# Niccolo-Ajroldi/plainLM

Hardware: AMD Instinct MI355X
Metric: tokens/sec fwd+bwd (160M, seq=1024, bf16) (higher is better)
Workload: dtype bf16

## Files before the change

### plainlm_amd/csrc/attn_causal.hip

```cpp
#include "plm_device.h"

#include <type_traits>

#include "attn_common.h"

template <int RB>
__device__ __forceinline__ void attn_block2(int T, int nh, int& tile, int& h, int& b) {
  const int ntile = (T + RB - 1) / RB;
  const int nbh = gridDim.x / ntile;
  const int bh = blockIdx.x % nbh;
  tile = blockIdx.x / nbh;
  h = bh % nh;
  b = bh / nh;
}

constexpr int ATTN_DMA_PER_STAGE = 4;
constexpr int ATTN_DMA_STATS = 2;
static_assert(ATTN_DMA_PER_STAGE == 2 * 2, "stage() = two TileDma::issue calls of two instructions each");

#define ATTN_DEFER_LOG2 8.0f
#define PLM_ATTN_TRACE_SETTER plm_dbg_attn_trace_causal
ATTN_TRACE_DECL()
#ifdef PLM_ATTN_ONEPASS_ABLATION
static __device__ float* g_onepass_buf = nullptr;
static __device__ int g_onepass_mode = 0;
extern "C" int plm_dbg_attn_onepass(float* buf, int mode) {
  if (hipMemcpyToSymbol(HIP_SYMBOL(g_onepass_buf), &buf, sizeof(buf)) != hipSuccess) return -1;
  return (int)hipMemcpyToSymbol(HIP_SYMBOL(g_onepass_mode), &mode, sizeof(mode));
}
#define ONEPASS_LDS 8192
#else
#define ONEPASS_LDS 0
#endif

enum { QB_OFF = 0, QB_UM = 1, QB_MASK = 2 };

template <int NST>
__global__ __launch_bounds__(256, 2) void attn_fwd_causal_kernel(const uint16_t* __restrict__ qkv, uint16_t* __restrict__ out,
                                                                 float* __restrict__ lse, int T, int nh) {
  constexpr int KT = 64;
  constexpr int TILE = KT * 128;
  constexpr int QB = 256;
  __shared__ __attribute__((aligned(1024))) char smem[NST * 2 * TILE];

  int tile_, h, b;
  attn_block2<QB>(T, nh, tile_, h, b);
  const int qt = (T + QB - 1) / QB - 1 - tile_;
  const int dm = nh * HD, ld = 3 * dm;
  const int t = threadIdx.x, lane = t & 63;
  const int wave = __builtin_amdgcn_readfirstlane(t >> 6);
  const int l31 = lane & 31, hi = lane >> 5;
  const int q0 = qt * QB;
  const int r0[2] = {q0 + 32 * wave, q0 + 32 * (7 - wave)};
  const uint16_t* base = qkv + (int64_t)b * T * ld + h * HD;
  const float c2 = 0.125f * LOG2E;

  const int kv_hi = min(T, q0 + QB);
  const int jt_hi = (kv_hi + KT - 1) / KT;
  constexpr int jt_lo = 0;
  const int n = jt_hi;

  TileDma dma;
  dma.init(wave, lane, ld);
  auto stage = [&](int slot, int jt) {
    const int kv0 = jt * KT;
    const uint16_t* src = base + (int64_t)kv0 * ld;
    if (kv0 + KT <= T) {
      dma.issue_full(smem + slot * 2 * TILE, src + dm, wave);
      dma.issue_full(smem + slot * 2 * TILE + TILE, src + 2 * dm, wave);
    } else {
      dma.issue(smem + slot * 2 * TILE, src + dm, ld, T - 1 - kv0, wave);
      dma.issue(smem + slot * 2 * TILE + TILE, src + 2 * dm, ld, T - 1 - kv0, wave);
    }
  };

  if (n > 0) stage(0, jt_lo);

  bf16x8_t qf[2][4];
#pragma unroll
  for (int qb = 0; qb < 2; ++qb) {
    const int qrow = r0[qb] + l31;
    const bool qvalid = qrow < T;
#pragma unroll
    for (int ks = 0; ks < 4; ++ks) qf[qb][ks] = qvalid ? ld_bf16x8(base + (int64_t)qrow * ld + ks * 16 + hi * 8) : zero_bf16x8();
  }
#pragma unroll
  for (int qb = 0; qb < 2; ++qb) asm volatile("; q fragments resident" ::"v"(qf[qb][0]), "v"(qf[qb][1]), "v"(qf[qb][2]), "v"(qf[qb][3]));
  asm volatile("s_waitcnt vmcnt(0)" ::: "memory");
#pragma unroll
  for (int i = 1; i < NST - 1; ++i)
    if (i < n) stage(i, jt_lo + i);

  f32x16_t o[2][2];
  float mc[2], lsum[2];
#pragma unroll
  for (int qb = 0; qb < 2; ++qb) {
    zero16(o[qb][0]);
    zero16(o[qb][1]);
    mc[qb] = -INFINITY;
    lsum[qb] = 0.f;
  }

  auto soft_pv = [&](int qb_, f32x16_t (&s)[2], const bf16x8_t (&vfr)[2][4], int kv0, auto mask_tag) {
    constexpr bool MASK = decltype(mask_tag)::value;
    const int qb = qb_;
    const int c_hi = r0[qb] + l31 - kv0 - 4 * hi;
    float tmax = -INFINITY;
#pragma unroll
    for (int kb = 0; kb < 2; ++kb)
#pragma unroll
      for (int r = 0; r < 16; ++r) {
        if (MASK) {
          const int c = kb * 32 + (r & 3) + 8 * (r >> 2);
          if (c > c_hi) s[kb][r] = -INFINITY;
        }
        tmax = fmaxf(tmax, s[kb][r]);
      }
    {
      float t_lo, t_hi;
      half_pair(tmax, t_lo, t_hi);
      tmax = fmaxf(t_lo, t_hi);
    }
    const float tm = tmax * c2;
    const bool need = tm > mc[qb] + ATTN_DEFER_LOG2;
    if (__builtin_amdgcn_ballot_w64(need) != 0ull) {
      const float mn = fmaxf(mc[qb], tm);
      const float alpha = fast_exp2(mc[qb] - ((mn == -INFINITY) ? 0.f : mn));
      mc[qb] = mn;
      lsum[qb] *= alpha;
#pragma unroll
      for (int db = 0; db < 2; ++db)
#pragma unroll
        for (int r = 0; r < 16; ++r) o[qb][db][r] *= alpha;
    }
    const float mref = (MASK && mc[qb] == -INFINITY) ? 0.f : mc[qb];
    float ps[4] = {0.f, 0.f, 0.f, 0.f};
    bf16x8_t pf[4];
#pragma unroll
    for (int kb = 0; kb < 2; ++kb)
#pragma unroll
      for (int r = 0; r < 16; ++r) {
        const float p = fast_exp2(__builtin_fmaf(s[kb][r], c2, -mref));
        ps[r & 3] += p;
        pf[kb * 2 + (r >> 3)][r & 7] = f2bf(p);
      }
    lsum[qb] += (ps[0] + ps[1]) + (ps[2] + ps[3]);
#pragma unroll
    for (int db = 0; db < 2; ++db)
#pragma unroll
      for (int sp = 0; sp < 4; ++sp) o[qb][db] = mfma32(vfr[db][sp], pf[sp], o[qb][db]);
  };

  auto compute = [&](int kv0, const char* sK, const char* sV, auto m0_tag, auto m1_tag) {
    constexpr int M0 = decltype(m0_tag)::value, M1 = decltype(m1_tag)::value;
    bf16x8_t kfr[2][4];
#pragma unroll
    for (int kb = 0; kb < 2; ++kb)
#pragma unroll
      for (int ks = 0; ks < 4; ++ks) kfr[kb][ks] = frag_rows(sK, kb * 32 + l31, ks, hi);
    f32x16_t s[2][2];
#pragma unroll
    for (int qb = 0; qb < 2; ++qb) {
      if ((qb == 0 ? M0 : M1) == QB_OFF) continue;
#pragma unroll
      for (int kb = 0; kb < 2; ++kb) {
        zero16(s[qb][kb]);
#pragma unroll
        for (int ks = 0; ks < 4; ++ks) s[qb][kb] = mfma32(kfr[kb][ks], qf[qb][ks], s[qb][kb]);
      }
    }
    __builtin_amdgcn_sched_barrier(0);
    bf16x8_t vfr[2][4];
#pragma unroll
    for (int db = 0; db < 2; ++db)
#pragma unroll
      for (int sp = 0; sp < 4; ++sp) vfr[db][sp] = frag_cols(sV, db, (sp >> 1) * 32 + (sp & 1) * 16 + 4 * hi, lane);
    if (M0 == QB_UM) soft_pv(0, s[0], vfr, kv0, std::false_type{});
    if (M0 == QB_MASK) soft_pv(0, s[0], vfr, kv0, std::true_type{});
    if (M1 == QB_UM) soft_pv(1, s[1], vfr, kv0, std::false_type{});
    if (M1 == QB_MASK) soft_pv(1, s[1], vfr, kv0, std::true_type{});
  };

  int i = 0, slot = 0;
  auto run = [&](int jt_end, auto m0_tag, auto m1_tag, bool active) {
    for (; jt_lo + i < jt_end; ++i) {
      const int rem = min(NST - 2, n - 1 - i);
      if (NST >= 4 && rem >= 2) attn_wait_vm<2 * ATTN_DMA_PER_STAGE>();
      else if (NST >= 3 && rem == 1) attn_wait_vm<ATTN_DMA_PER_STAGE>();
      else attn_wait_vm<0>();
      attn_barrier();
      if (i + NST - 1 < n) stage(slot == 0 ? NST - 1 : slot - 1, jt_lo + i + NST - 1);
      if (active) compute((jt_lo + i) * KT, smem + slot * 2 * TILE, smem + slot * 2 * TILE + TILE, m0_tag, m1_tag);
      slot = (slot + 1 == NST) ? 0 : slot + 1;
    }
  };
  using OFF_ = std::integral_constant<int, QB_OFF>;
  using UM_ = std::integral_constant<int, QB_UM>;
  using MK_ = std::integral_constant<int, QB_MASK>;
  const int a0 = min(jt_hi, r0[0] / KT), e0 = min(jt_hi, r0[0] / KT + 1);
  const int a1 = min(jt_hi, r0[1] / KT), e1 = min(jt_hi, r0[1] / KT + 1);
  run(a0, UM_{}, UM_{}, true);
  run(e0, MK_{}, UM_{}, true);
  run(a1, OFF_{}, UM_{}, true);
  run(e1, OFF_{}, MK_{}, true);
  run(jt_hi, OFF_{}, OFF_{}, false);

  const RowStage rs{smem + (n % NST) * 2 * TILE + wave * 4096, lane};
#pragma unroll
  for (int qb = 0; qb < 2; ++qb) {
    const int qrow = r0[qb] + l31;
    float l_lo, l_hi;
    half_pair(lsum[qb], l_lo, l_hi);
    const float ltot = l_lo + l_hi;
    const float inv = 1.f / ltot;
#pragma unroll
    for (int db = 0; db < 2; ++db)
#pragma unroll
      for (int g = 0; g < 4; ++g) {
        bf16x4_t v;
#pragma unroll
        for (int e = 0; e < 4; ++e) v[e] = f2bf(o[qb][db][4 * g + e] * inv);
        rs.put(l31, hi, db * 4 + g, v);
      }
    if (qrow < T && hi == 0) lse[((int64_t)b * nh + h) * T + qrow] = mc[qb] + __builtin_amdgcn_logf(ltot);
    rs.flush(out + (int64_t)b * T * dm, dm, r0[qb], T, h * HD);
  }
}

template <int NST>
__global__ __launch_bounds__(256, 2) void attn_bwd_dq_causal_kernel(const uint16_t* __restrict__ qkv, const uint16_t* __restrict__ out,
                                                              const uint16_t* __restrict__ dout, const float* __restrict__ lse,
                                                              float* __restrict__ delta, const float* __restrict__ rcos,
                                                              const float* __restrict__ rsin, uint16_t* __restrict__ dqkv, int T, int nh,
                                                              float dsign) {
  constexpr int KT = 64;
  constexpr int TILE = KT * 128;
  constexpr int QB = 256;
  __shared__ __attribute__((aligned(1024))) char smem[NST * 2 * TILE];

  int tile_, h, b;
  attn_block2<QB>(T, nh, tile_, h, b);
  const int qt = (T + QB - 1) / QB - 1 - tile_;
  const int dm = nh * HD, ld = 3 * dm;
  const int t = threadIdx.x, lane = t & 63;
  const int wave = __builtin_amdgcn_readfirstlane(t >> 6);
  const int l31 = lane & 31, hi = lane >> 5;
  const int q0 = qt * QB;
  const int r0[2] = {q0 + 32 * wave, q0 + 32 * (7 - wave)};
  const uint16_t* base = qkv + (int64_t)b * T * ld + h * HD;
  const float scale = 0.125f, c2 = scale * LOG2E;

  const int kv_hi = min(T, q0 + QB);
  const int jt_hi = (kv_hi + KT - 1) / KT;
  constexpr int jt_lo = 0;
  const int n = jt_hi;

  TileDma dma;
  dma.init(wave, lane, ld);
  auto stage = [&](int slot, int jt) {
    const int kv0 = jt * KT;
    const uint16_t* src = base + (int64_t)kv0 * ld;
    if (kv0 + KT <= T) {
      dma.issue_full(smem + slot * 2 * TILE, src + dm, wave);
      dma.issue_full(smem + slot * 2 * TILE + TILE, src + 2 * dm, wave);
    } else {
      dma.issue(smem + slot * 2 * TILE, src + dm, ld, T - 1 - kv0, wave);
      dma.issue(smem + slot * 2 * TILE + TILE, src + 2 * dm, ld, T - 1 - kv0, wave);
    }
  };

  if (n > 0) stage(0, jt_lo);

  bf16x8_t qf[2][4], dof[2][4];
  float Lq[2], Dq[2];
#pragma unroll
  for (int qb = 0; qb < 2; ++qb) {
    const int qrow = r0[qb] + l31;
    const bool qvalid = qrow < T;
#pragma unroll
    for (int ks = 0; ks < 4; ++ks) {
      const int d0 = ks * 16 + hi * 8;
      qf[qb][ks] = qvalid ? ld_bf16x8(base + (int64_t)qrow * ld + d0) : zero_bf16x8();
      dof[qb][ks] = qvalid ? ld_bf16x8(dout + ((int64_t)b * T + qrow) * dm + h * HD + d0) : zero_bf16x8();
    }
    Lq[qb] = 0.f;
    float part = 0.f;
    if (qvalid) {
      Lq[qb] = lse[((int64_t)b * nh + h) * T + qrow];
#pragma unroll
      for (int ks = 0; ks < 4; ++ks) {
        const bf16x8_t o8 = ld_bf16x8(out + ((int64_t)b * T + qrow) * dm + h * HD + ks * 16 + hi * 8);
#pragma unroll
        for (int e = 0; e < 8; ++e) part += bf2f(o8[e]) * bf2f(dof[qb][ks][e]);
      }
    }
    float d_lo, d_hi;
    half_pair(part, d_lo, d_hi);
    Dq[qb] = d_lo + d_hi;
  }
#pragma unroll
  for (int qb = 0; qb < 2; ++qb)
    asm volatile("; q/dO fragments resident" ::"v"(qf[qb][0]), "v"(qf[qb][1]), "v"(qf[qb][2]), "v"(qf[qb][3]), "v"(dof[qb][0]), "v"(dof[qb][1]),
                 "v"(dof[qb][2]), "v"(dof[qb][3]), "v"(Lq[qb]), "v"(Dq[qb]));
  asm volatile("s_waitcnt vmcnt(0)" ::: "memory");
#pragma unroll
  for (int i = 1; i < NST - 1; ++i)
    if (i < n) stage(i, jt_lo + i);

  f32x16_t dq[2][2];
#pragma unroll
  for (int qb = 0; qb < 2; ++qb) {
    zero16(dq[qb][0]);
    zero16(dq[qb][1]);
  }

  auto block = [&](int qb_, int kb, const bf16x8_t (&kfr)[4], const bf16x8_t (&vfr)[4], const bf16x8_t (&ktr)[2][2], int kv0, auto mask_tag) {
    constexpr bool MASK = decltype(mask_tag)::value;
    const int qb = qb_;
    const int c_hi = r0[qb] + l31 - kv0 - 4 * hi;
    f32x16_t s, dp;
    zero16(s);
    zero16(dp);
#pragma unroll
    for (int ks = 0; ks < 4; ++ks) {
      s = mfma32(kfr[ks], qf[qb][ks], s);
      dp = mfma32(vfr[ks], dof[qb][ks], dp);
    }
    bf16x8_t dsf[2];
#pragma unroll
    for (int r = 0; r < 16; ++r) {
      float p = fast_exp2(__builtin_fmaf(s[r], c2, -Lq[qb]));
      if (MASK) {
        const int c = kb * 32 + (r & 3) + 8 * (r >> 2);
        p = (c <= c_hi) ? p : 0.f;
      }
      dsf[r >> 3][r & 7] = f2bf(p * (dp[r] - Dq[qb]));
    }
#pragma unroll
    for (int s2 = 0; s2 < 2; ++s2)
#pragma unroll
      for (int db = 0; db < 2; ++db) dq[qb][db] = mfma32(ktr[db][s2], dsf[s2], dq[qb][db]);
  };

  auto compute = [&](int kv0, const char* sK, const char* sV, auto m0_tag, auto m1_tag) {
    constexpr int M0 = decltype(m0_tag)::value, M1 = decltype(m1_tag)::value;
#pragma unroll
    for (int kb = 0; kb < 2; ++kb) {
      __builtin_amdgcn_sched_barrier(0);
      bf16x8_t kfr[4], vfr[4], ktr[2][2];
#pragma unroll
      for (int ks = 0; ks < 4; ++ks) {
        kfr[ks] = frag_rows(sK, kb * 32 + l31, ks, hi);
        vfr[ks] = frag_rows(sV, kb * 32 + l31, ks, hi);
      }
#pragma unroll
      for (int s2 = 0; s2 < 2; ++s2)
#pragma unroll
        for (int db = 0; db < 2; ++db) ktr[db][s2] = frag_cols(sK, db, kb * 32 + s2 * 16 + 4 * hi, lane);
      if (M0 == QB_UM) block(0, kb, kfr, vfr, ktr, kv0, std::false_type{});
      if (M0 == QB_MASK) block(0, kb, kfr, vfr, ktr, kv0, std::true_type{});
      if (M1 == QB_UM) block(1, kb, kfr, vfr, ktr, kv0, std::false_type{});
      if (M1 == QB_MASK) block(1, kb, kfr, vfr, ktr, kv0, std::true_type{});
    }
  };

  int i = 0, slot = 0;
  auto run = [&](int jt_end, auto m0_tag, auto m1_tag, bool active) {
    for (; jt_lo + i < jt_end; ++i) {
      const int rem = min(NST - 2, n - 1 - i);
      if (NST >= 4 && rem >= 2) attn_wait_vm<2 * ATTN_DMA_PER_STAGE>();
      else if (NST >= 3 && rem == 1) attn_wait_vm<ATTN_DMA_PER_STAGE>();
      else attn_wait_vm<0>();
      attn_barrier();
      if (i + NST - 1 < n) stage(slot == 0 ? NST - 1 : slot - 1, jt_lo + i + NST - 1);
      if (active) compute((jt_lo + i) * KT, smem + slot * 2 * TILE, smem + slot * 2 * TILE + TILE, m0_tag, m1_tag);
      slot = (slot + 1 == NST) ? 0 : slot + 1;
    }
  };
  using OFF_ = std::integral_constant<int, QB_OFF>;
  using UM_ = std::integral_constant<int, QB_UM>;
  using MK_ = std::integral_constant<int, QB_MASK>;
  const int a0 = min(jt_hi, r0[0] / KT), e0 = min(jt_hi, r0[0] / KT + 1);
  const int a1 = min(jt_hi, r0[1] / KT), e1 = min(jt_hi, r0[1] / KT + 1);
  run(a0, UM_{}, UM_{}, true);
  run(e0, MK_{}, UM_{}, true);
  run(a1, OFF_{}, UM_{}, true);
  run(e1, OFF_{}, MK_{}, true);
  run(jt_hi, OFF_{}, OFF_{}, false);

  const RowStage rs{smem + (n % NST) * 2 * TILE + wave * 4096, lane};
#pragma unroll
  for (int qb = 0; qb < 2; ++qb) {
    if (r0[qb] + l31 < T && hi == 0) delta[((int64_t)b * nh + h) * T + r0[qb] + l31] = Dq[qb] * dsign;
#pragma unroll
    for (int db = 0; db < 2; ++db)
#pragma unroll
      for (int g = 0; g < 4; ++g) {
        bf16x4_t ov;
#pragma unroll
        for (int e = 0; e < 4; ++e) ov[e] = f2bf(dq[qb][db][4 * g + e] * scale);
        rs.put(l31, hi, db * 4 + g, ov);
      }
    rs.flush_rot(dqkv + (int64_t)b * T * ld, ld, r0[qb], T, h * HD, rcos, rsin);
  }
}

template <int NST, bool DOC>
__device__ __forceinline__ void attn_bwd_dkdv_body(char* smem, const uint16_t* __restrict__ qkv, const uint16_t* __restrict__ dout,
                                                   const float* __restrict__ lse, const float* __restrict__ ndelta,
                                                   const float* __restrict__ rcos, const float* __restrict__ rsin,
                                                   const int32_t* __restrict__ doc_end, uint16_t* __restrict__ dqkv, int T, int nh, int b, int h,
                                                   int kv0, int jq_plan, unsigned long long* trace_t = nullptr) {
  constexpr int QT = 64;
  constexpr int TILE = QT * 128;
  constexpr int STAGE = 2 * TILE + 512;
  constexpr int NQB = 2;
  const int dm = nh * HD, ld = 3 * dm;
  const int t = threadIdx.x, lane = t & 63;
  const int wave = __builtin_amdgcn_readfirstlane(t >> 6);
  const int l31 = lane & 31, hi = lane >> 5;
  constexpr int qoff = 0;
  const int kvw0 = kv0 + 32 * wave;
  const int kvrow = kvw0 + l31;
  const bool kvalid = kvrow < T;
  const uint16_t* base = qkv + (int64_t)b * T * ld + h * HD;
  const uint16_t* dobase = dout + (int64_t)b * T * dm + h * HD;
  const float* lrow = lse + ((int64_t)b * nh + h) * T;
  const float* drow = ndelta + ((int64_t)b * nh + h) * T;
  const float scale = 0.125f, c2 = scale * LOG2E;

  const int nqt = (T + QT - 1) / QT;
  const int jq_lo = kv0 / QT;
  const int jq_hi = DOC ? jq_plan : nqt;
  const int n = jq_hi - jq_lo;

  TileDma dma, dmad;
  dma.init(wave, lane, ld);
  dmad.init(wave, lane, dm);
  auto stage = [&](int slot, int jq) {
    const int qt0 = jq * QT;
    char* dst = smem + slot * STAGE;
    if (qt0 + QT <= T) {
      dma.issue_full(dst, base + (int64_t)qt0 * ld, wave);
      dmad.issue_full(dst + TILE, dobase + (int64_t)qt0 * dm, wave);
    } else {
      dma.issue(dst, base + (int64_t)qt0 * ld, ld, T - 1 - qt0, wave);
      dma.issue(dst + TILE, dobase + (int64_t)qt0 * dm, dm, T - 1 - qt0, wave);
    }
    if (wave == 0 && lane < 16) {
      const int q = min(qt0 + lane * 4, T - 4);
      dma16_asm(lrow + q, dst + 2 * TILE);
      dma16_asm(drow + q, dst + 2 * TILE + 256);
    }
  };
  bf16x8_t kf[4], vf[4];
  int de = T;
  if (DOC) {
    static_assert(!DOC || NST == 3, "the prologue parks the wave's rows in slots 1 and 2");
    if (n > 0) stage(0, jq_lo);
    char* kreg = smem + 1 * STAGE + wave * 4096;
    char* vreg = smem + 2 * STAGE + wave * 4096;
    rows_dma(kreg, base + dm, ld, kvw0, T - 1, lane);
    rows_dma(vreg, base + 2 * dm, ld, kvw0, T - 1, lane);
    de = doc_end[(int64_t)b * T + min(kvrow, T - 1)];
    asm volatile("; row data requested" ::"v"(de));
    asm volatile("s_waitcnt vmcnt(0)" ::: "memory");
#pragma unroll
    for (int ks = 0; ks < 4; ++ks) {
      kf[ks] = rows_frag(kreg, l31, ks, hi);
      vf[ks] = rows_frag(vreg, l31, ks, hi);
    }
    attn_barrier();
    if (n > 1) stage(1, jq_lo + 1);
  } else {
#pragma unroll
    for (int i = 0; i < NST - 1; ++i)
      if (i < n) stage(i, jq_lo + i);
#pragma unroll
    for (int ks = 0; ks < 4; ++ks) {
      const uint16_t* p = base + (int64_t)kvrow * ld + ks * 16 + hi * 8;
      kf[ks] = kvalid ? ld_bf16x8(p + dm) : zero_bf16x8();
      vf[ks] = kvalid ? ld_bf16x8(p + 2 * dm) : zero_bf16x8();
    }
    asm volatile("; k/v fragments resident" ::"v"(kf[0]), "v"(kf[1]), "v"(kf[2]), "v"(kf[3]), "v"(vf[0]), "v"(vf[1]), "v"(vf[2]), "v"(vf[3]));
    asm volatile("s_waitcnt vmcnt(0)" ::: "memory");
  }
  const int de_lo = DOC ? __builtin_amdgcn_readlane(de, 0) : T, de_hi = DOC ? __builtin_amdgcn_readlane(de, 31) : T;

  f32x16_t dk[2], dv[2];
  zero16(dk[0]); zero16(dk[1]); zero16(dv[0]); zero16(dv[1]);

  auto compute = [&](int qt0, const char* sQ, auto mask_tag) {
    constexpr bool MASK = decltype(mask_tag)::value;
    const char* sDO = sQ + TILE;
    const float* sL = reinterpret_cast<const float*>(sQ + 2 * TILE);
    const float* sD = sL + 64;
    const int c_lo = kvrow - qt0 - qoff - 4 * hi, c_end = de - qt0 - qoff - 4 * hi;
#pragma unroll
    for (int qb = 0; qb < NQB; ++qb) {
      __builtin_amdgcn_sched_barrier(0);
      if (MASK && qt0 + qoff + qb * 32 + 31 < kvw0) continue;
      if (DOC && MASK && qt0 + qoff + qb * 32 >= de_hi) continue;
      bf16x8_t qfr[4], dofr[4], dotr[2][2], qtr[2][2];
#pragma unroll
      for (int ks = 0; ks < 4; ++ks) {
        qfr[ks] = frag_rows(sQ, qoff + qb * 32 + l31, ks, hi);
        dofr[ks] = frag_rows(sDO, qoff + qb * 32 + l31, ks, hi);
      }
      f32x4_t L4[4];
      f32x16_t s, dp;
#pragma unroll
      for (int g = 0; g < 4; ++g) {
        const int ql0 = qoff + qb * 32 + 8 * g + 4 * hi;
        L4[g] = *reinterpret_cast<const f32x4_t*>(sL + ql0);
        const f32x4_t nd = *reinterpret_cast<const f32x4_t*>(sD + ql0);
#pragma unroll
        for (int e = 0; e < 4; ++e) dp[4 * g + e] = nd[e];
      }
#pragma unroll
      for (int s2 = 0; s2 < 2; ++s2)
#pragma unroll
        for (int db = 0; db < 2; ++db) {
          dotr[db][s2] = frag_cols(sDO, db, qoff + qb * 32 + s2 * 16 + 4 * hi, lane);
          qtr[db][s2] = frag_cols(sQ, db, qoff + qb * 32 + s2 * 16 + 4 * hi, lane);
        }
      zero16(s);
#pragma unroll
      for (int ks = 0; ks < 4; ++ks) {
        s = mfma32(qfr[ks], kf[ks], s);
        dp = mfma32(dofr[ks], vf[ks], dp);
      }
      bf16x8_t pf[2], dsf[2];
#pragma unroll
      for (int g = 0; g < 4; ++g)
#pragma unroll
        for (int e = 0; e < 4; ++e) {
          const int r = 4 * g + e;
          float p = fast_exp2(__builtin_fmaf(s[r], c2, -L4[g][e]));
          if (MASK) {
            const int c = qb * 32 + 8 * g + e;
            p = ((c >= c_lo) && (c < c_end)) ? p : 0.f;
          }
          const float dsv = p * dp[r];
          pf[r >> 3][r & 7] = f2bf(p);
          dsf[r >> 3][r & 7] = f2bf(dsv);
        }
#pragma unroll
      for (int s2 = 0; s2 < 2; ++s2)
#pragma unroll
        for (int db = 0; db < 2; ++db) {
          dv[db] = mfma32(dotr[db][s2], pf[s2], dv[db]);
          dk[db] = mfma32(qtr[db][s2], dsf[s2], dk[db]);
        }
#ifdef PLM_ATTN_ONEPASS_ABLATION
      if (g_onepass_mode) {
        char* scr = smem + NST * STAGE + wave * 2048;
        *reinterpret_cast<bf16x8_t*>(scr + lane * 32) = dsf[0];
        *reinterpret_cast<bf16x8_t*>(scr + lane * 32 + 16) = dsf[1];
        bf16x8_t at[2];
#pragma unroll
        for (int s2 = 0; s2 < 2; ++s2)
          at[s2] = join_tr(lds_read_tr16(scr + s2 * 1024 + (lane & 15) * 64 + (lane >> 4) * 8), lds_read_tr16(scr + s2 * 1024 + 512 + (lane & 15) * 32 + (lane >> 4) * 8));
        f32x16_t dqp[2];
        zero16(dqp[0]);
        zero16(dqp[1]);
#pragma unroll
        for (int s2 = 0; s2 < 2; ++s2)
#pragma unroll
          for (int db = 0; db < 2; ++db) dqp[db] = mfma32(at[s2], frag_cols(sQ, db, qoff + qb * 32 + s2 * 16 + 4 * hi, lane), dqp[db]);
        if (g_onepass_mode == 2) {
#pragma unroll
          for (int db = 0; db < 2; ++db)
#pragma unroll
            for (int r = 0; r < 16; ++r) {
              const int q = min(qt0 + qb * 32 + mfma32_row(r, hi), T - 1);
              atomicAdd(g_onepass_buf + ((int64_t)b * T + q) * dm + h * HD + db * 32 + l31, dqp[db][r]);
            }
        } else {
          asm volatile("; partial dQ" ::"v"(dqp[0]), "v"(dqp[1]));
        }
      }
#endif
    }
  };

  const bool wave_rows = kvw0 < T;
  const int jq_act = wave_rows ? min(jq_hi, max(jq_lo, kvw0 / QT)) : jq_hi;
  const int jq_m = min(jq_hi, max(jq_act, (kvw0 + 31 + QT - 1) / QT));
  const int jq_u = min(jq_hi, max(jq_m, de_lo / QT));
  const int jq_e = min(jq_hi, max(jq_u, (de_hi + QT - 1) / QT));
#ifdef PLM_ATTN_TRACE
  if (trace_t) trace_t[0] = __builtin_amdgcn_s_memrealtime();
#endif
  int i = 0, slot = 0;
  auto run = [&](int jq_end, auto mask_tag, bool active) {
    for (; jq_lo + i < jq_end; ++i) {
      const int rem = min(NST - 2, n - 1 - i);
      constexpr int W0 = ATTN_DMA_PER_STAGE + ATTN_DMA_STATS;
      if (wave == 0) {
        if (NST >= 4 && rem >= 2) attn_wait_vm<2 * W0>();
        else if (NST >= 3 && rem == 1) attn_wait_vm<W0>();
        else attn_wait_vm<0>();
      } else {
        if (NST >= 4 && rem >= 2) attn_wait_vm<2 * ATTN_DMA_PER_STAGE>();
        else if (NST >= 3 && rem == 1) attn_wait_vm<ATTN_DMA_PER_STAGE>();
        else attn_wait_vm<0>();
      }
      attn_barrier();
      if (i + NST - 1 < n) stage(slot == 0 ? NST - 1 : slot - 1, jq_lo + i + NST - 1);
      if (active) compute((jq_lo + i) * QT, smem + slot * STAGE, mask_tag);
      slot = (slot + 1 == NST) ? 0 : slot + 1;
    }
  };
  run(jq_act, std::true_type{}, false);
  run(jq_m, std::true_type{}, true);
  run(jq_u, std::false_type{}, true);
  run(jq_e, std::true_type{}, true);
  if (DOC) run(jq_hi, std::true_type{}, false);
#ifdef PLM_ATTN_TRACE
  if (trace_t) trace_t[1] = __builtin_amdgcn_s_memrealtime();
#endif

  const RowStage rs{smem + (n % NST) * STAGE + wave * 4096, lane};
#pragma unroll
  for (int db = 0; db < 2; ++db)
#pragma unroll
    for (int g = 0; g < 4; ++g) {
      bf16x4_t ov;
#pragma unroll
      for (int e = 0; e < 4; ++e) ov[e] = f2bf(dv[db][4 * g + e]);
      rs.put(l31, hi, db * 4 + g, ov);
    }
  rs.flush(dqkv + (int64_t)b * T * ld, ld, kvw0, T, 2 * dm + h * HD);
#pragma unroll
  for (int db = 0; db < 2; ++db)
#pragma unroll
    for (int g = 0; g < 4; ++g) {
      bf16x4_t ok;
#pragma unroll
      for (int e = 0; e < 4; ++e) ok[e] = f2bf(dk[db][4 * g + e] * scale);
      rs.put(l31, hi, db * 4 + g, ok);
    }
  rs.flush_rot(dqkv + (int64_t)b * T * ld, ld, kvw0, T, dm + h * HD, rcos, rsin);
}


template <int NST>
__global__ __launch_bounds__(256, 2) void attn_bwd_dkdv_causal_kernel(const uint16_t* __restrict__ qkv, const uint16_t* __restrict__ dout,
                                                                      const float* __restrict__ lse, const float* __restrict__ ndelta,
                                                                      const float* __restrict__ rcos, const float* __restrict__ rsin,
                                                                      uint16_t* __restrict__ dqkv, int T, int nh) {
  __shared__ __attribute__((aligned(1024))) char smem[NST * (2 * 8192 + 512) + ONEPASS_LDS];
  int kt, h, b;
  attn_block2<128>(T, nh, kt, h, b);
  attn_bwd_dkdv_body<NST, false>(smem, qkv, dout, lse, ndelta, rcos, rsin, nullptr, dqkv, T, nh, b, h, kt * 128, 0);
}

template <int NST>
__global__ __launch_bounds__(256, 2) void attn_bwd_dkdv_doc_kernel(const uint16_t* __restrict__ qkv, const uint16_t* __restrict__ dout,
                                                                   const float* __restrict__ lse, const float* __restrict__ ndelta,
                                                                   const float* __restrict__ rcos, const float* __restrict__ rsin,
                                                                   const int32_t* __restrict__ header, const int32_t* __restrict__ doc_end,
                                                                   const int4* __restrict__ items, uint16_t* __restrict__ dqkv, int T, int nh) {
  __shared__ __attribute__((aligned(1024))) char smem[NST * (2 * 8192 + 512) + ONEPASS_LDS];
  ATTN_TRACE_T(tr0);
  const int idx = blockIdx.x / nh, h = blockIdx.x - idx * nh;
  if (idx >= __builtin_amdgcn_readfirstlane(header[0])) return;
  const int4 it = items[idx];
  const int b = __builtin_amdgcn_readfirstlane(it.x), kv0 = __builtin_amdgcn_readfirstlane(it.y), jq_hi = __builtin_amdgcn_readfirstlane(it.z);
  const int kc = __builtin_amdgcn_readfirstlane(it.w);
  (void)kc;
#ifdef PLM_ATTN_TRACE
  unsigned long long tt[2] = {0, 0};
#else
  unsigned long long* tt = nullptr;
#endif
  attn_bwd_dkdv_body<NST, true>(smem, qkv, dout, lse, ndelta, rcos, rsin, doc_end, dqkv, T, nh, b, h, kv0, jq_hi, tt);
  ATTN_TRACE_END(2, idx, kc, tr0, tt[0], tt[1]);
}

void plm_attn_fwd_causal(const uint16_t* qkv, uint16_t* out, float* lse, int64_t B, int64_t T, int64_t nh, hipStream_t s) {
  const dim3 grid((unsigned)(plm_cdiv(T, 256) * nh * B)), block(256);
  hipLaunchKernelGGL((attn_fwd_causal_kernel<4>), grid, block, 0, s, qkv, out, lse, (int)T, (int)nh);
}
void plm_attn_bwd_causal(const uint16_t* qkv, const uint16_t* out, const uint16_t* dout, const float* lse, float* delta, const float* rc,
                         const float* rs, uint16_t* dqkv, int64_t B, int64_t T, int64_t nh, hipStream_t s) {
  const dim3 block(256);
  hipLaunchKernelGGL((attn_bwd_dq_causal_kernel<3>), dim3((unsigned)(plm_cdiv(T, 256) * nh * B)), block, 0, s, qkv, out, dout, lse, delta, rc, rs, dqkv, (int)T, (int)nh, -1.f);
  hipLaunchKernelGGL((attn_bwd_dkdv_causal_kernel<3>), dim3((unsigned)(plm_cdiv(T, 128) * nh * B)), block, 0, s, qkv, dout, lse, delta, rc, rs, dqkv,
                     (int)T, (int)nh);
}
void plm_attn_bwd_dkdv_doc(const uint16_t* qkv, const uint16_t* dout, const float* lse, const float* ndelta, const float* rc, const float* rs,
                           const int32_t* header, const int32_t* doc_end, const int4* items_k, uint16_t* dqkv, int64_t B, int64_t T, int64_t nh,
                           hipStream_t s) {
  hipLaunchKernelGGL((attn_bwd_dkdv_doc_kernel<3>), dim3((unsigned)(doc_plan_cap(B, T) * nh)), dim3(256), 0, s, qkv, dout, lse, ndelta, rc, rs,
                     header, doc_end, items_k, dqkv, (int)T, (int)nh);
}
```

### plainlm_amd/csrc/attn_common.h

```cpp
#pragma once
#include "plm_device.h"

#define HD 64
#define LOG2E 1.4426950408889634f

__device__ __forceinline__ float fast_exp2(float x) { return __builtin_amdgcn_exp2f(x); }

__device__ __forceinline__ int rs_off(int row, int c) {
  const int pp = ((c >> 1) + 2 * ((row >> 1) & 1) + ((row >> 3) & 1)) & 3;
  const int ph = (c & 1) ^ ((row >> 2) & 1);
  return row * 128 + pp * 32 + ph * 16;
}
__device__ __forceinline__ int rs_logical_chunk(int row, int pc) {
  const int cb = ((pc >> 1) - 2 * ((row >> 1) & 1) - ((row >> 3) & 1)) & 3;
  return cb * 2 + ((pc & 1) ^ ((row >> 2) & 1));
}

__device__ __forceinline__ bf16x8_t frag_rows(const char* tile, int row, int ks, int hi) {
  return *reinterpret_cast<const bf16x8_t*>(tile + rs_off(row, ks * 2 + hi));
}
__device__ __forceinline__ bf16x8_t frag_cols(const char* tile, int db, int rbase, int lane) {
  const int ib = (lane >> 4) & 1, t16 = lane & 15;
  const int sub = t16 & 3;
  const int c = (db * 2 + ib) * 2 + (sub >> 1);
  const int row = rbase + (t16 >> 2);
  const char* p0 = tile + rs_off(row, c) + (sub & 1) * 8;
  const char* p1 = tile + rs_off(row + 8, c) + (sub & 1) * 8;
  return join_tr(lds_read_tr16(p0), lds_read_tr16(p1));
}

struct TileDma {
  int row[2], coff[2];
  unsigned boff[2];
  __device__ __forceinline__ void init(int wave, int lane, int64_t ld = 0) {
#pragma unroll
    for (int i = 0; i < 2; ++i) {
      row[i] = (i * 4 + wave) * 8 + (lane >> 3);
      coff[i] = rs_logical_chunk(row[i], lane & 7) * 8;
      boff[i] = (unsigned)((row[i] * ld + coff[i]) * 2);
    }
  }
  __device__ __forceinline__ void issue(char* dst_tile, const uint16_t* src, int64_t ld, int last_row, int wave, int row0 = 0) const {
#pragma unroll
    for (int i = 0; i < 2; ++i)
      dma16_asm(src + (int64_t)min(row0 + row[i], last_row) * ld + coff[i], dst_tile + (i * 4 + wave) * 1024);
  }
  __device__ __forceinline__ void issue_full(char* dst_tile, const uint16_t* src, int wave) const {
#pragma unroll
    for (int i = 0; i < 2; ++i) dma16_saddr_asm(src, boff[i], dst_tile + (i * 4 + wave) * 1024);
  }
};

__device__ __forceinline__ void rows_dma(char* region, const uint16_t* src, int64_t ld, int row0, int last_row, int lane) {
#pragma unroll
  for (int i = 0; i < 4; ++i) {
    const int row = 8 * i + (lane >> 3);
    dma16_asm(src + (int64_t)min(row0 + row, last_row) * ld + rs_logical_chunk(row, lane & 7) * 8, region + i * 1024);
  }
}
__device__ __forceinline__ bf16x8_t rows_frag(const char* region, int l31, int ks, int hi) {
  return *reinterpret_cast<const bf16x8_t*>(region + rs_off(l31, ks * 2 + hi));
}

template <int N>
__device__ __forceinline__ void attn_wait_vm() {
  asm volatile("s_waitcnt vmcnt(%0)" ::"n"(N) : "memory");
}
__device__ __forceinline__ void attn_barrier() { asm volatile("s_waitcnt lgkmcnt(0)\n\ts_barrier" ::: "memory"); }

__device__ __forceinline__ void zero16(f32x16_t& v) {
#pragma unroll
  for (int r = 0; r < 16; ++r) v[r] = 0.f;
}

struct RowStage {
  char* base;
  int lane;
  __device__ __forceinline__ void put(int l31, int hi, int c16, bf16x4_t v) const {
    *reinterpret_cast<bf16x4_t*>(base + l31 * 128 + ((c16 ^ (l31 & 7)) << 4) + hi * 8) = v;
  }
  __device__ __forceinline__ void flush(uint16_t* dst, int64_t ld, int row0, int row_end, int col0) const {
#pragma unroll
    for (int i = 0; i < 4; ++i) {
      const int row = 8 * i + (lane >> 3), c16 = lane & 7;
      const bf16x8_t v = *reinterpret_cast<const bf16x8_t*>(base + row * 128 + ((c16 ^ (row & 7)) << 4));
      if (row0 + row < row_end) st_bf16x8(dst + (int64_t)(row0 + row) * ld + col0 + c16 * 8, v);
    }
  }
  __device__ __forceinline__ void flush_rot(uint16_t* dst, int64_t ld, int row0, int row_end, int col0, const float* __restrict__ rcos,
                                            const float* __restrict__ rsin) const {
    f32x4_t cs[4], sn[4];
#pragma unroll
    for (int i = 0; i < 4; ++i) {
      const int trow = min(row0 + 8 * i + (lane >> 3), row_end - 1);
      cs[i] = *reinterpret_cast<const f32x4_t*>(rcos + trow * (HD / 2) + (lane & 7) * 4);
      sn[i] = *reinterpret_cast<const f32x4_t*>(rsin + trow * (HD / 2) + (lane & 7) * 4);
    }
#pragma unroll
    for (int i = 0; i < 4; ++i) {
      const int row = 8 * i + (lane >> 3), c16 = lane & 7;
      const bf16x8_t v = *reinterpret_cast<const bf16x8_t*>(base + row * 128 + ((c16 ^ (row & 7)) << 4));
      if (row0 + row < row_end) st_bf16x8(dst + (int64_t)(row0 + row) * ld + col0 + c16 * 8, rope8(v, cs[i], sn[i], -1.f));
    }
  }
};


struct DocPlan {
  const int32_t* header;
  const int32_t* doc_end;
  const int4* items_q;
  const int4* items_k;
};
constexpr int DOC_KIND_SHIFT = 30;
__host__ __device__ __forceinline__ int64_t doc_plan_tiles(int64_t B, int64_t T) { return B * ((T + 127) / 128); }
__host__ __device__ __forceinline__ int64_t doc_plan_cap(int64_t B, int64_t T) { return doc_plan_tiles(B, T) + doc_plan_tiles(B, T) / 4; }
__host__ __device__ __forceinline__ int64_t doc_plan_pq(int64_t B, int64_t T) { return (8 + B * T + 3) & ~(int64_t)3; }
__host__ __device__ __forceinline__ int64_t doc_plan_ints(int64_t B, int64_t T) { return doc_plan_pq(B, T) + 8 * doc_plan_cap(B, T); }
__host__ __device__ __forceinline__ DocPlan doc_plan_view(const int32_t* plan, int64_t B, int64_t T) {
  DocPlan p;
  p.header = plan;
  p.doc_end = plan + 8;
  p.items_q = reinterpret_cast<const int4*>(plan + doc_plan_pq(B, T));
  p.items_k = p.items_q + doc_plan_cap(B, T);
  return p;
}

#ifdef PLM_ATTN_TRACE
#define ATTN_TRACE_DECL()                                                                    \
  static __device__ unsigned long long* g_attn_trace = nullptr;                               \
  extern "C" int PLM_ATTN_TRACE_SETTER(unsigned long long* buf) {                             \
    return (int)hipMemcpyToSymbol(HIP_SYMBOL(g_attn_trace), &buf, sizeof(buf));               \
  }
#define ATTN_TRACE_T(var) const unsigned long long var = __builtin_amdgcn_s_memrealtime()
#define ATTN_TRACE_END(kid, rank_, cost_, t0, t1, t2)                                                                              \
  if (threadIdx.x == 0 && g_attn_trace) {                                                                                          \
    unsigned long long* r_ = g_attn_trace + ((size_t)(kid) * 65536 + blockIdx.x) * 8;                                             \
    r_[0] = t0; r_[1] = t1; r_[2] = t2; r_[3] = __builtin_amdgcn_s_memrealtime();                                                 \
    r_[4] = __builtin_amdgcn_s_getreg((31 << 11) | 4); r_[5] = __builtin_amdgcn_s_getreg((31 << 11) | 20);                         \
    r_[6] = (unsigned long long)(rank_); r_[7] = (unsigned long long)(cost_);                                                      \
  }
#else
#define ATTN_TRACE_DECL()
#define ATTN_TRACE_T(var)
#define ATTN_TRACE_END(kid, rank_, cost_, t0, t1, t2)
#endif
```

Before: 1.071 million.

## Switch causal attention backward kernels from 32x32 to 16x16 MFMA tiles

Rewrites the dQ and dK/dV causal backward kernels to use 16x16x32 MFMA instructions instead of 32x32x16, with new LDS fragment loaders (frag_rows16, frag_cols16, rows_frag16) and regrouped accumulators. The delta reduction now uses cross-lane shuffles, and masking and doc-end bounds are recomputed per 16-row subtile. The aim is better MFMA throughput or latency and finer masking granularity on MI355X. The cost is more instructions and more fragment loads, and the new lane-to-row mappings are easy to get wrong.

```diff
diff --git a/plainlm_amd/csrc/attn_causal.hip b/plainlm_amd/csrc/attn_causal.hip
--- a/plainlm_amd/csrc/attn_causal.hip
+++ b/plainlm_amd/csrc/attn_causal.hip
@@ -244,7 +244,7 @@
   const int dm = nh * HD, ld = 3 * dm;
   const int t = threadIdx.x, lane = t & 63;
   const int wave = __builtin_amdgcn_readfirstlane(t >> 6);
-  const int l31 = lane & 31, hi = lane >> 5;
+  const int l15 = lane & 15, g = lane >> 4;
   const int q0 = qt * QB;
   const int r0[2] = {q0 + 32 * wave, q0 + 32 * (7 - wave)};
   const uint16_t* base = qkv + (int64_t)b * T * ld + h * HD;
@@ -271,75 +271,86 @@
 
   if (n > 0) stage(0, jt_lo);
 
-  bf16x8_t qf[2][4], dof[2][4];
-  float Lq[2], Dq[2];
-#pragma unroll
-  for (int qb = 0; qb < 2; ++qb) {
-    const int qrow = r0[qb] + l31;
-    const bool qvalid = qrow < T;
-#pragma unroll
-    for (int ks = 0; ks < 4; ++ks) {
-      const int d0 = ks * 16 + hi * 8;
-      qf[qb][ks] = qvalid ? ld_bf16x8(base + (int64_t)qrow * ld + d0) : zero_bf16x8();
-      dof[qb][ks] = qvalid ? ld_bf16x8(dout + ((int64_t)b * T + qrow) * dm + h * HD + d0) : zero_bf16x8();
-    }
-    Lq[qb] = 0.f;
-    float part = 0.f;
-    if (qvalid) {
-      Lq[qb] = lse[((int64_t)b * nh + h) * T + qrow];
-#pragma unroll
-      for (int ks = 0; ks < 4; ++ks) {
-        const bf16x8_t o8 = ld_bf16x8(out + ((int64_t)b * T + qrow) * dm + h * HD + ks * 16 + hi * 8);
-#pragma unroll
-        for (int e = 0; e < 8; ++e) part += bf2f(o8[e]) * bf2f(dof[qb][ks][e]);
-      }
-    }
-    float d_lo, d_hi;
-    half_pair(part, d_lo, d_hi);
-    Dq[qb] = d_lo + d_hi;
-  }
+  bf16x8_t qf[2][2][2], dof[2][2][2];
+  float Lq[2][2], Dq[2][2];
 #pragma unroll
   for (int qb = 0; qb < 2; ++qb)
-    asm volatile("; q/dO fragments resident" ::"v"(qf[qb][0]), "v"(qf[qb][1]), "v"(qf[qb][2]), "v"(qf[qb][3]), "v"(dof[qb][0]), "v"(dof[qb][1]),
-                 "v"(dof[qb][2]), "v"(dof[qb][3]), "v"(Lq[qb]), "v"(Dq[qb]));
+#pragma unroll
+    for (int qt = 0; qt < 2; ++qt) {
+      const int qrow = r0[qb] + 16 * qt + l15;
+      const bool qvalid = qrow < T;
+#pragma unroll
+      for (int ks = 0; ks < 2; ++ks) {
+        const int d0 = ks * 32 + g * 8;
+        qf[qb][qt][ks] = qvalid ? ld_bf16x8(base + (int64_t)qrow * ld + d0) : zero_bf16x8();
+        dof[qb][qt][ks] = qvalid ? ld_bf16x8(dout + ((int64_t)b * T + qrow) * dm + h * HD + d0) : zero_bf16x8();
+      }
+      Lq[qb][qt] = 0.f;
+      float part = 0.f;
+      if (qvalid) {
+        Lq[qb][qt] = lse[((int64_t)b * nh + h) * T + qrow];
+#pragma unroll
+        for (int ks = 0; ks < 2; ++ks) {
+          const bf16x8_t o8 = ld_bf16x8(out + ((int64_t)b * T + qrow) * dm + h * HD + ks * 32 + g * 8);
+#pragma unroll
+          for (int e = 0; e < 8; ++e) part += bf2f(o8[e]) * bf2f(dof[qb][qt][ks][e]);
+        }
+      }
+      part += __shfl_xor(part, 16, 64);
+      part += __shfl_xor(part, 32, 64);
+      Dq[qb][qt] = part;
+    }
+#pragma unroll
+  for (int qb = 0; qb < 2; ++qb)
+#pragma unroll
+    for (int qt = 0; qt < 2; ++qt)
+      asm volatile("; q/dO fragments resident" ::"v"(qf[qb][qt][0]), "v"(qf[qb][qt][1]), "v"(dof[qb][qt][0]), "v"(dof[qb][qt][1]), "v"(Lq[qb][qt]),
+                   "v"(Dq[qb][qt]));
   asm volatile("s_waitcnt vmcnt(0)" ::: "memory");
 #pragma unroll
   for (int i = 1; i < NST - 1; ++i)
     if (i < n) stage(i, jt_lo + i);
 
-  f32x16_t dq[2][2];
-#pragma unroll
-  for (int qb = 0; qb < 2; ++qb) {
-    zero16(dq[qb][0]);
-    zero16(dq[qb][1]);
-  }
-
-  auto block = [&](int qb_, int kb, const bf16x8_t (&kfr)[4], const bf16x8_t (&vfr)[4], const bf16x8_t (&ktr)[2][2], int kv0, auto mask_tag) {
+  f32x4_t dq[2][2][4];
+#pragma unroll
+  for (int qb = 0; qb < 2; ++qb)
+#pragma unroll
+    for (int qt = 0; qt < 2; ++qt)
+#pragma unroll
+      for (int dt = 0; dt < 4; ++dt) zero4(dq[qb][qt][dt]);
+
+  auto block = [&](int qb_, int kb, const bf16x8_t (&kfr)[2][2], const bf16x8_t (&vfr)[2][2], const bf16x8_t (&ktr)[4], int kv0, auto mask_tag) {
     constexpr bool MASK = decltype(mask_tag)::value;
     const int qb = qb_;
-    const int c_hi = r0[qb] + l31 - kv0 - 4 * hi;
-    f32x16_t s, dp;
-    zero16(s);
-    zero16(dp);
-#pragma unroll
-    for (int ks = 0; ks < 4; ++ks) {
-      s = mfma32(kfr[ks], qf[qb][ks], s);
-      dp = mfma32(vfr[ks], dof[qb][ks], dp);
-    }
-    bf16x8_t dsf[2];
-#pragma unroll
-    for (int r = 0; r < 16; ++r) {
-      float p = fast_exp2(__builtin_fmaf(s[r], c2, -Lq[qb]));
-      if (MASK) {
-        const int c = kb * 32 + (r & 3) + 8 * (r >> 2);
-        p = (c <= c_hi) ? p : 0.f;
-      }
-      dsf[r >> 3][r & 7] = f2bf(p * (dp[r] - Dq[qb]));
-    }
-#pragma unroll
-    for (int s2 = 0; s2 < 2; ++s2)
-#pragma unroll
-      for (int db = 0; db < 2; ++db) dq[qb][db] = mfma32(ktr[db][s2], dsf[s2], dq[qb][db]);
+#pragma unroll
+    for (int qt = 0; qt < 2; ++qt) {
+      const int c_hi = r0[qb] + 16 * qt + l15 - kv0 - 8 * g;
+      f32x4_t s[2], dp[2];
+#pragma unroll
+      for (int kh = 0; kh < 2; ++kh) {
+        zero4(s[kh]);
+        zero4(dp[kh]);
+#pragma unroll
+        for (int ks = 0; ks < 2; ++ks) {
+          s[kh] = mfma16(kfr[kh][ks], qf[qb][qt][ks], s[kh]);
+          dp[kh] = mfma16(vfr[kh][ks], dof[qb][qt][ks], dp[kh]);
+        }
+      }
+      bf16x8_t dsf;
+#pragma unroll
+      for (int kh = 0; kh < 2; ++kh)
+#pragma unroll
+        for (int r = 0; r < 4; ++r) {
+          float p = fast_exp2(__builtin_fmaf(s[kh][r], c2, -Lq[qb][qt]));
+          if (MASK) {
+            const int c = kb * 32 + 4 * kh + r;
+            p = (c <= c_hi) ? p : 0.f;
+          }
+          dsf[4 * kh + r] = f2bf(p * (dp[kh][r] - Dq[qb][qt]));
+        }
+#pragma unroll
+      for (int dt = 0; dt < 4; ++dt) dq[qb][qt][dt] = mfma16(ktr[dt], dsf, dq[qb][qt][dt]);
+    }
   };
 
   auto compute = [&](int kv0, const char* sK, const char* sV, auto m0_tag, auto m1_tag) {
@@ -347,16 +358,16 @@
 #pragma unroll
     for (int kb = 0; kb < 2; ++kb) {
       __builtin_amdgcn_sched_barrier(0);
-      bf16x8_t kfr[4], vfr[4], ktr[2][2];
-#pragma unroll
-      for (int ks = 0; ks < 4; ++ks) {
-        kfr[ks] = frag_rows(sK, kb * 32 + l31, ks, hi);
-        vfr[ks] = frag_rows(sV, kb * 32 + l31, ks, hi);
-      }
-#pragma unroll
-      for (int s2 = 0; s2 < 2; ++s2)
-#pragma unroll
-        for (int db = 0; db < 2; ++db) ktr[db][s2] = frag_cols(sK, db, kb * 32 + s2 * 16 + 4 * hi, lane);
+      bf16x8_t kfr[2][2], vfr[2][2], ktr[4];
+#pragma unroll
+      for (int kh = 0; kh < 2; ++kh)
+#pragma unroll
+        for (int ks = 0; ks < 2; ++ks) {
+          kfr[kh][ks] = frag_rows16(sK, kb * 32, kh, ks, lane);
+          vfr[kh][ks] = frag_rows16(sV, kb * 32, kh, ks, lane);
+        }
+#pragma unroll
+      for (int dt = 0; dt < 4; ++dt) ktr[dt] = frag_cols16(sK, dt, kb * 32, lane);
       if (M0 == QB_UM) block(0, kb, kfr, vfr, ktr, kv0, std::false_type{});
       if (M0 == QB_MASK) block(0, kb, kfr, vfr, ktr, kv0, std::true_type{});
       if (M1 == QB_UM) block(1, kb, kfr, vfr, ktr, kv0, std::false_type{});
@@ -391,16 +402,18 @@
   const RowStage rs{smem + (n % NST) * 2 * TILE + wave * 4096, lane};
 #pragma unroll
   for (int qb = 0; qb < 2; ++qb) {
-    if (r0[qb] + l31 < T && hi == 0) delta[((int64_t)b * nh + h) * T + r0[qb] + l31] = Dq[qb] * dsign;
-#pragma unroll
-    for (int db = 0; db < 2; ++db)
-#pragma unroll
-      for (int g = 0; g < 4; ++g) {
+#pragma unroll
+    for (int qt = 0; qt < 2; ++qt) {
+      const int qrow = r0[qb] + 16 * qt + l15;
+      if (qrow < T && g == 0) delta[((int64_t)b * nh + h) * T + qrow] = Dq[qb][qt] * dsign;
+#pragma unroll
+      for (int dt = 0; dt < 4; ++dt) {
         bf16x4_t ov;
 #pragma unroll
-        for (int e = 0; e < 4; ++e) ov[e] = f2bf(dq[qb][db][4 * g + e] * scale);
-        rs.put(l31, hi, db * 4 + g, ov);
-      }
+        for (int e = 0; e < 4; ++e) ov[e] = f2bf(dq[qb][qt][dt][e] * scale);
+        rs.put(16 * qt + l15, g & 1, dt * 2 + (g >> 1), ov);
+      }
+    }
     rs.flush_rot(dqkv + (int64_t)b * T * ld, ld, r0[qb], T, h * HD, rcos, rsin);
   }
 }
@@ -418,11 +431,10 @@
   const int dm = nh * HD, ld = 3 * dm;
   const int t = threadIdx.x, lane = t & 63;
   const int wave = __builtin_amdgcn_readfirstlane(t >> 6);
-  const int l31 = lane & 31, hi = lane >> 5;
+  const int l15 = lane & 15, g = lane >> 4;
   constexpr int qoff = 0;
   const int kvw0 = kv0 + 32 * wave;
-  const int kvrow = kvw0 + l31;
-  const bool kvalid = kvrow < T;
+  const int kvrow = kvw0 + l15;
   const uint16_t* base = qkv + (int64_t)b * T * ld + h * HD;
   const uint16_t* dobase = dout + (int64_t)b * T * dm + h * HD;
   const float* lrow = lse + ((int64_t)b * nh + h) * T;
@@ -453,8 +465,8 @@
       dma16_asm(drow + q, dst + 2 * TILE + 256);
     }
   };
-  bf16x8_t kf[4], vf[4];
-  int de = T;
+  bf16x8_t kf[2][2], vf[2][2];
+  int de[2] = {T, T};
   if (DOC) {
     static_assert(!DOC || NST == 3, "the prologue parks the wave's rows in slots 1 and 2");
     if (n > 0) stage(0, jq_lo);
@@ -462,14 +474,17 @@
     char* vreg = smem + 2 * STAGE + wave * 4096;
     rows_dma(kreg, base + dm, ld, kvw0, T - 1, lane);
     rows_dma(vreg, base + 2 * dm, ld, kvw0, T - 1, lane);
-    de = doc_end[(int64_t)b * T + min(kvrow, T - 1)];
-    asm volatile("; row data requested" ::"v"(de));
+    de[0] = doc_end[(int64_t)b * T + min(kvrow, T - 1)];
+    de[1] = doc_end[(int64_t)b * T + min(kvrow + 16, T - 1)];
+    asm volatile("; row data requested" ::"v"(de[0]), "v"(de[1]));
     asm volatile("s_waitcnt vmcnt(0)" ::: "memory");
 #pragma unroll
-    for (int ks = 0; ks < 4; ++ks) {
-      kf[ks] = rows_frag(kreg, l31, ks, hi);
-      vf[ks] = rows_frag(vreg, l31, ks, hi);
-    }
+    for (int kt = 0; kt < 2; ++kt)
+#pragma unroll
+      for (int ks = 0; ks < 2; ++ks) {
+        kf[kt][ks] = rows_frag16(kreg, kt, ks, lane);
+        vf[kt][ks] = rows_frag16(vreg, kt, ks, lane);
+      }
     attn_barrier();
     if (n > 1) stage(1, jq_lo + 1);
   } else {
@@ -477,83 +492,101 @@
     for (int i = 0; i < NST - 1; ++i)
       if (i < n) stage(i, jq_lo + i);
 #pragma unroll
-    for (int ks = 0; ks < 4; ++ks) {
-      const uint16_t* p = base + (int64_t)kvrow * ld + ks * 16 + hi * 8;
-      kf[ks] = kvalid ? ld_bf16x8(p + dm) : zero_bf16x8();
-      vf[ks] = kvalid ? ld_bf16x8(p + 2 * dm) : zero_bf16x8();
-    }
-    asm volatile("; k/v fragments resident" ::"v"(kf[0]), "v"(kf[1]), "v"(kf[2]), "v"(kf[3]), "v"(vf[0]), "v"(vf[1]), "v"(vf[2]), "v"(vf[3]));
+    for (int kt = 0; kt < 2; ++kt)
+#pragma unroll
+      for (int ks = 0; ks < 2; ++ks) {
+        const bool kvalid = kvrow + 16 * kt < T;
+        const uint16_t* p = base + (int64_t)(kvrow + 16 * kt) * ld + ks * 32 + g * 8;
+        kf[kt][ks] = kvalid ? ld_bf16x8(p + dm) : zero_bf16x8();
+        vf[kt][ks] = kvalid ? ld_bf16x8(p + 2 * dm) : zero_bf16x8();
+      }
+    asm volatile("; k/v fragments resident" ::"v"(kf[0][0]), "v"(kf[0][1]), "v"(kf[1][0]), "v"(kf[1][1]), "v"(vf[0][0]), "v"(vf[0][1]), "v"(vf[1][0]),
+                 "v"(vf[1][1]));
     asm volatile("s_waitcnt vmcnt(0)" ::: "memory");
   }
-  const int de_lo = DOC ? __builtin_amdgcn_readlane(de, 0) : T, de_hi = DOC ? __builtin_amdgcn_readlane(de, 31) : T;
-
-  f32x16_t dk[2], dv[2];
-  zero16(dk[0]); zero16(dk[1]); zero16(dv[0]); zero16(dv[1]);
+  const int de_lo = DOC ? __builtin_amdgcn_readlane(de[0], 0) : T, de_hi = DOC ? __builtin_amdgcn_readlane(de[1], 15) : T;
+
+  f32x4_t dk[4][2], dv[4][2];
+#pragma unroll
+  for (int dt = 0; dt < 4; ++dt)
+#pragma unroll
+    for (int kt = 0; kt < 2; ++kt) {
+      zero4(dk[dt][kt]);
+      zero4(dv[dt][kt]);
+    }
 
   auto compute = [&](int qt0, const char* sQ, auto mask_tag) {
     constexpr bool MASK = decltype(mask_tag)::value;
     const char* sDO = sQ + TILE;
     const float* sL = reinterpret_cast<const float*>(sQ + 2 * TILE);
     const float* sD = sL + 64;
-    const int c_lo = kvrow - qt0 - qoff - 4 * hi, c_end = de - qt0 - qoff - 4 * hi;
+    const int c_lo = kvrow - qt0 - qoff - 8 * g;
+    const int c_end[2] = {de[0] - qt0 - qoff - 8 * g, de[1] - qt0 - qoff - 8 * g};
 #pragma unroll
     for (int qb = 0; qb < NQB; ++qb) {
       __builtin_amdgcn_sched_barrier(0);
       if (MASK && qt0 + qoff + qb * 32 + 31 < kvw0) continue;
       if (DOC && MASK && qt0 + qoff + qb * 32 >= de_hi) continue;
-      bf16x8_t qfr[4], dofr[4], dotr[2][2], qtr[2][2];
-#pragma unroll
-      for (int ks = 0; ks < 4; ++ks) {
-        qfr[ks] = frag_rows(sQ, qoff + qb * 32 + l31, ks, hi);
-        dofr[ks] = frag_rows(sDO, qoff + qb * 32 + l31, ks, hi);
-      }
-      f32x4_t L4[4];
-      f32x16_t s, dp;
-#pragma unroll
-      for (int g = 0; g < 4; ++g) {
-        const int ql0 = qoff + qb * 32 + 8 * g + 4 * hi;
-        L4[g] = *reinterpret_cast<const f32x4_t*>(sL + ql0);
+      bf16x8_t qfr[2][2], dofr[2][2], dotr[4], qtr[4];
+#pragma unroll
+      for (int qh = 0; qh < 2; ++qh)
+#pragma unroll
+        for (int ks = 0; ks < 2; ++ks) {
+          qfr[qh][ks] = frag_rows16(sQ, qoff + qb * 32, qh, ks, lane);
+          dofr[qh][ks] = frag_rows16(sDO, qoff + qb * 32, qh, ks, lane);
+        }
+      f32x4_t L4[2];
+      f32x4_t s[2][2], dp[2][2];
+#pragma unroll
+      for (int qh = 0; qh < 2; ++qh) {
+        const int ql0 = qoff + qb * 32 + 8 * g + 4 * qh;
+        L4[qh] = *reinterpret_cast<const f32x4_t*>(sL + ql0);
         const f32x4_t nd = *reinterpret_cast<const f32x4_t*>(sD + ql0);
-#pragma unroll
-        for (int e = 0; e < 4; ++e) dp[4 * g + e] = nd[e];
-      }
-#pragma unroll
-      for (int s2 = 0; s2 < 2; ++s2)
-#pragma unroll
-        for (int db = 0; db < 2; ++db) {
-          dotr[db][s2] = frag_cols(sDO, db, qoff + qb * 32 + s2 * 16 + 4 * hi, lane);
-          qtr[db][s2] = frag_cols(sQ, db, qoff + qb * 32 + s2 * 16 + 4 * hi, lane);
-        }
-      zero16(s);
-#pragma unroll
-      for (int ks = 0; ks < 4; ++ks) {
-        s = mfma32(qfr[ks], kf[ks], s);
-        dp = mfma32(dofr[ks], vf[ks], dp);
-      }
+        dp[qh][0] = nd;
+        dp[qh][1] = nd;
+      }
+#pragma unroll
+      for (int dt = 0; dt < 4; ++dt) {
+        dotr[dt] = frag_cols16(sDO, dt, qoff + qb * 32, lane);
+        qtr[dt] = frag_cols16(sQ, dt, qoff + qb * 32, lane);
+      }
+#pragma unroll
+      for (int qh = 0; qh < 2; ++qh)
+#pragma unroll
+        for (int kt = 0; kt < 2; ++kt) {
+          zero4(s[qh][kt]);
+#pragma unroll
+          for (int ks = 0; ks < 2; ++ks) {
+            s[qh][kt] = mfma16(qfr[qh][ks], kf[kt][ks], s[qh][kt]);
+            dp[qh][kt] = mfma16(dofr[qh][ks], vf[kt][ks], dp[qh][kt]);
+          }
+        }
       bf16x8_t pf[2], dsf[2];
 #pragma unroll
-      for (int g = 0; g < 4; ++g)
-#pragma unroll
-        for (int e = 0; e < 4; ++e) {
-          const int r = 4 * g + e;
-          float p = fast_exp2(__builtin_fmaf(s[r], c2, -L4[g][e]));
-          if (MASK) {
-            const int c = qb * 32 + 8 * g + e;
-            p = ((c >= c_lo) && (c < c_end)) ? p : 0.f;
+      for (int kt = 0; kt < 2; ++kt)
+#pragma unroll
+        for (int qh = 0; qh < 2; ++qh)
+#pragma unroll
+          for (int e = 0; e < 4; ++e) {
+            float p = fast_exp2(__builtin_fmaf(s[qh][kt][e], c2, -L4[qh][e]));
+            if (MASK) {
+              const int c = qb * 32 + 4 * qh + e;
+              p = ((c >= c_lo + 16 * kt) && (c < c_end[kt])) ? p : 0.f;
+            }
+            const float dsv = p * dp[qh][kt][e];
+            pf[kt][4 * qh + e] = f2bf(p);
+            dsf[kt][4 * qh + e] = f2bf(dsv);
           }
-          const float dsv = p * dp[r];
-          pf[r >> 3][r & 7] = f2bf(p);
-          dsf[r >> 3][r & 7] = f2bf(dsv);
-        }
-#pragma unroll
-      for (int s2 = 0; s2 < 2; ++s2)
-#pragma unroll
-        for (int db = 0; db < 2; ++db) {
-          dv[db] = mfma32(dotr[db][s2], pf[s2], dv[db]);
-          dk[db] = mfma32(qtr[db][s2], dsf[s2], dk[db]);
+#pragma unroll
+      for (int dt = 0; dt < 4; ++dt)
+#pragma unroll
+        for (int kt = 0; kt < 2; ++kt) {
+          dv[dt][kt] = mfma16(dotr[dt], pf[kt], dv[dt][kt]);
+          dk[dt][kt] = mfma16(qtr[dt], dsf[kt], dk[dt][kt]);
         }
 #ifdef PLM_ATTN_ONEPASS_ABLATION
       if (g_onepass_mode) {
+        const int l31 = lane & 31, hi = lane >> 5;
         char* scr = smem + NST * STAGE + wave * 2048;
         *reinterpret_cast<bf16x8_t*>(scr + lane * 32) = dsf[0];
         *reinterpret_cast<bf16x8_t*>(scr + lane * 32 + 16) = dsf[1];
@@ -623,23 +656,23 @@
 
   const RowStage rs{smem + (n % NST) * STAGE + wave * 4096, lane};
 #pragma unroll
-  for (int db = 0; db < 2; ++db)
-#pragma unroll
-    for (int g = 0; g < 4; ++g) {
+  for (int kt = 0; kt < 2; ++kt)
+#pragma unroll
+    for (int dt = 0; dt < 4; ++dt) {
       bf16x4_t ov;
 #pragma unroll
-      for (int e = 0; e < 4; ++e) ov[e] = f2bf(dv[db][4 * g + e]);
-      rs.put(l31, hi, db * 4 + g, ov);
+      for (int e = 0; e < 4; ++e) ov[e] = f2bf(dv[dt][kt][e]);
+      rs.put(16 * kt + l15, g & 1, dt * 2 + (g >> 1), ov);
     }
   rs.flush(dqkv + (int64_t)b * T * ld, ld, kvw0, T, 2 * dm + h * HD);
 #pragma unroll
-  for (int db = 0; db < 2; ++db)
-#pragma unroll
-    for (int g = 0; g < 4; ++g) {
+  for (int kt = 0; kt < 2; ++kt)
+#pragma unroll
+    for (int dt = 0; dt < 4; ++dt) {
       bf16x4_t ok;
 #pragma unroll
-      for (int e = 0; e < 4; ++e) ok[e] = f2bf(dk[db][4 * g + e] * scale);
-      rs.put(l31, hi, db * 4 + g, ok);
+      for (int e = 0; e < 4; ++e) ok[e] = f2bf(dk[dt][kt][e] * scale);
+      rs.put(16 * kt + l15, g & 1, dt * 2 + (g >> 1), ok);
     }
   rs.flush_rot(dqkv + (int64_t)b * T * ld, ld, kvw0, T, dm + h * HD, rcos, rsin);
 }
diff --git a/plainlm_amd/csrc/attn_common.h b/plainlm_amd/csrc/attn_common.h
--- a/plainlm_amd/csrc/attn_common.h
+++ b/plainlm_amd/csrc/attn_common.h
@@ -26,6 +26,19 @@
   const int row = rbase + (t16 >> 2);
   const char* p0 = tile + rs_off(row, c) + (sub & 1) * 8;
   const char* p1 = tile + rs_off(row + 8, c) + (sub & 1) * 8;
+  return join_tr(lds_read_tr16(p0), lds_read_tr16(p1));
+}
+
+__device__ __forceinline__ int tile16_row(int i, int half) { return 8 * (i >> 2) + 4 * half + (i & 3); }
+__device__ __forceinline__ bf16x8_t frag_rows16(const char* tile, int rbase, int half, int ks, int lane) {
+  return *reinterpret_cast<const bf16x8_t*>(tile + rs_off(rbase + tile16_row(lane & 15, half), ks * 4 + (lane >> 4)));
+}
+__device__ __forceinline__ bf16x8_t frag_cols16(const char* tile, int dt, int rbase, int lane) {
+  const int t16 = lane & 15, sub = t16 & 3;
+  const int c = dt * 2 + (sub >> 1);
+  const int row = rbase + 8 * (lane >> 4) + (t16 >> 2);
+  const char* p0 = tile + rs_off(row, c) + (sub & 1) * 8;
+  const char* p1 = tile + rs_off(row + 4, c) + (sub & 1) * 8;
   return join_tr(lds_read_tr16(p0), lds_read_tr16(p1));
 }
 
@@ -62,6 +75,10 @@
   return *reinterpret_cast<const bf16x8_t*>(region + rs_off(l31, ks * 2 + hi));
 }
 
+__device__ __forceinline__ bf16x8_t rows_frag16(const char* region, int kt, int ks, int lane) {
+  return *reinterpret_cast<const bf16x8_t*>(region + rs_off(16 * kt + (lane & 15), ks * 4 + (lane >> 4)));
+}
+
 template <int N>
 __device__ __forceinline__ void attn_wait_vm() {
   asm volatile("s_waitcnt vmcnt(%0)" ::"n"(N) : "memory");
@@ -71,6 +88,11 @@
 __device__ __forceinline__ void zero16(f32x16_t& v) {
 #pragma unroll
   for (int r = 0; r < 16; ++r) v[r] = 0.f;
+}
+
+__device__ __forceinline__ void zero4(f32x4_t& v) {
+#pragma unroll
+  for (int r = 0; r < 4; ++r) v[r] = 0.f;
 }
 
 struct RowStage {
```

Result: no change. 1.074 million (median of 6 runs) (+0.3%).
